# BimberLab/nimble

Measured on NVIDIA B200. Metric: reads/sec (device-timed, 1/2/4/8 B200) vs MHC-like lib; SW GCUPS; HBM GB/s, higher is better.
Workload: dtype u64 k-mers / s16x2 DPX / f64 thresholds

## Files before the change

### nimble_b200/csrc/kernels.cuh

```cuda
#pragma once
#include <cstddef>
#include <cstdint>
#include <cuda_runtime.h>

#include "../../include/nimble_b200.h"
#include "kmer_hash.hpp"

namespace nb200 {

constexpr int kBand = 8;
constexpr int kNB = 2 * kBand + 1;
constexpr int kVW = 64;
constexpr uint32_t kXP = 0xFF7FFF7Fu;
constexpr uint32_t kGP = 0xFF3FFF3Fu;
constexpr uint32_t kMatchDelta = 193;
constexpr uint32_t kInvalid = 0xFFFFFFFFu;
constexpr int kCap = 32;
constexpr int kScratchWords = 16 * kCap;
constexpr uint32_t kFull = 0xFFFFFFFFu;
constexpr int kProbeWarps = 2;

struct LibDev {
    const uint4 *table;
    uint32_t n_buckets;
// ... 479 lines not shown
};

__device__ __forceinline__ bool candidate_round(const LibDev &lib, const int o, const uint32_t cl, uint32_t cap, int lane, uint32_t *lw, uint32_t *lb,
                                                int &na, int &owner, bool &dead, OwnerB &B) {
    const bool hit = cl != kInvalid;
    uint4 c_b, c_w;
    ldg256_cached(lib.class_rec + 2 * (size_t)(hit ? cl : 0u), c_b, c_w);
    const bool inl = (int32_t)c_w.z >= 0;
    if (na < 0) {
        const uint32_t cn = inl ? (c_w.z & 0xFFu) : c_b.y;
        const uint32_t m = __reduce_min_sync(kFull, hit ? ((min(cn, 0x3FFFFFFu) << 5) | (uint32_t)lane) : kInvalid);
        const int src = (int)(m & 31);
        const uint32_t nn = m >> 5;
        if (nn > cap) return false;
        na = (int)nn;
        if (nn <= 4 && owner < 0) {
            owner = o;
            B.w01 = __shfl_sync(kFull, c_w.x, src); B.w23 = __shfl_sync(kFull, c_w.y, src);
            B.b0 = __shfl_sync(kFull, c_b.x, src); B.b1 = __shfl_sync(kFull, c_b.y, src);
            B.b2 = __shfl_sync(kFull, c_b.z, src); B.b3 = __shfl_sync(kFull, c_b.w, src);
        } else {
            anchor_to_list(lib, lw, lb, nn, c_b, c_w, src, lane);
        }
    }
    if (o == owner) {
        const bool same = !hit || (c_w.x == B.w01 && c_w.y == B.w23 && inl);
        if (__all_sync(kFull, same)) {
            if (hit) { B.a0 &= c_b.x; B.a1 &= c_b.y; B.a2 &= c_b.z; B.a3 &= c_b.w; }
        } else {
            if (hit && inl) {
                B.a0 &= rec_bits(lib, c_b, c_w, B.w01 & 0xFFFFu);
                B.a1 &= rec_bits(lib, c_b, c_w, B.w01 >> 16);
                B.a2 &= rec_bits(lib, c_b, c_w, B.w23 & 0xFFFFu);
                B.a3 &= rec_bits(lib, c_b, c_w, B.w23 >> 16);
            }
            bool ovf = hit && !inl;
            while (__any_sync(kFull, ovf)) {
                if (ovf) {
#pragma unroll 1
                    for (int j = 0; j < na; j++) {
                        const uint32_t word = j == 0 ? (B.w01 & 0xFFFFu) : (j == 1 ? (B.w01 >> 16) : (j == 2 ? (B.w23 & 0xFFFFu) : (B.w23 >> 16)));
                        const uint32_t v = rec_lookup_overflow(lib.ov_w, lib.ov_b, c_b.x, c_b.y, word);
                        if (j == 0) B.a0 &= v; else if (j == 1) B.a1 &= v; else if (j == 2) B.a2 &= v; else B.a3 &= v;
                    }
                }
                ovf = false;
            }
        }
    } else if (!intersect_generic(lib, lw, lb, na, hit, c_b, c_w, lane)) {
        dead = true;
    }
    return true;
}

template <bool kStats>
__device__ __forceinline__ bool probe_mate(const LibDev &lib, const ReadsDev &R, uint64_t read, int lane, uint32_t cap,
                                           List *lists , MateProbe &M, uint32_t &n_probe, uint32_t &slots_read) {
    const uint8_t *rec = R.packed + read * R.stride;
    const int W = (int)R.words;
    const int L = read_length(R, read);
    const int k = lib.k;
    const int P = L - k + 1;
    M.L = L; M.P = P;
    const uint32_t kmask_lo = (uint32_t)lib.kmask, kmask_hi = (uint32_t)(lib.kmask >> 32), kbits = (uint32_t)lib.kbits;
    const int rshift = 64 - 2 * k;
    const uint32_t nb = lib.n_buckets;
    uint32_t nh0 = 0, nh1 = 0;
    int seed_i0 = -1, seed_i1 = -1;
    int na0 = -1, na1 = -1, owner = -1;
    bool dead0 = false, dead1 = false;
    OwnerB B;
    B.w01 = B.w23 = 0xFFFFFFFFu; B.b0 = B.b1 = B.b2 = B.b3 = 0; B.a0 = B.a1 = B.a2 = B.a3 = kFull;
    uint32_t my_lo = 0, my_hi = 0, my_n = 0;
    if (lane < W && P > 0) {
        const uint2 v = *reinterpret_cast<const uint2 *>(rec + (size_t)lane * 8);
        my_lo = v.x; my_hi = v.y;
        my_n = *reinterpret_cast<const uint32_t *>(rec + (size_t)W * 8 + (size_t)lane * 4);
    }
    uint32_t w0 = __shfl_sync(kFull, my_lo, 0), w1 = __shfl_sync(kFull, my_hi, 0), n_lo = __shfl_sync(kFull, my_n, 0);
    const bool upper = lane >= 16;
    const int n_rounds = P > 0 ? (P + 31) >> 5 : 0;

#pragma unroll 1
    for (int r = 0; r < n_rounds; r++) {
        const int i = (r << 5) + lane;
        const uint32_t w2 = __shfl_sync(kFull, my_lo, r + 1), w3 = __shfl_sync(kFull, my_hi, r + 1), n_hi = __shfl_sync(kFull, my_n, r + 1);
        const uint32_t ea = upper ? w1 : w0, eb = upper ? w2 : w1, ec = upper ? w3 : w2;
        const uint32_t x_lo = __funnelshift_r(ea, eb, 2 * lane) & kmask_lo;
        const uint32_t x_hi = __funnelshift_r(eb, ec, 2 * lane) & kmask_hi;
        const bool valid = i < P && (__funnelshift_r(n_lo, n_hi, lane) & kbits) == 0;
        w0 = w2; w1 = w3; n_lo = n_hi;
        uint32_t p_lo = __brev(~x_hi), p_hi = __brev(~x_lo);
        p_lo = ((p_lo >> 1) & 0x55555555u) | ((p_lo << 1) & 0xAAAAAAAAu);
        p_hi = ((p_hi >> 1) & 0x55555555u) | ((p_hi << 1) & 0xAAAAAAAAu);
        const uint32_t y_lo = rshift >= 32 ? p_hi >> (rshift - 32) : __funnelshift_r(p_lo, p_hi, rshift);
        const uint32_t y_hi = rshift >= 32 ? 0u : p_hi >> rshift;
        const bool x_lt = x_hi < y_hi || (x_hi == y_hi && x_lo < y_lo), x_eq = x_hi == y_hi && x_lo == y_lo;
        const uint32_t c_lo = x_lt ? x_lo : y_lo, c_hi = x_lt ? x_hi : y_hi;
        const uint32_t mix = kmer_mix(c_lo, c_hi);
        const uint32_t b1 = valid ? kmer_bucket1(mix, nb) : 0u;
        uint4 e_lo, e_hi;
        ldg256(lib.table + 2 * (size_t)b1, e_lo, e_hi);
        bool m0 = e_lo.x == c_lo && e_lo.y == c_hi, m1 = e_hi.x == c_lo && e_hi.y == c_hi;
        const bool need2 = valid && !(m0 || m1) && (e_lo.z & kDevSpill);
        if (kStats) { n_probe += valid ? 1u : 0u; slots_read += (valid ? 1u : 0u) + (need2 ? 1u : 0u); }
        const bool xs = x_lt || x_eq, ys = !x_lt;
        uint32_t ecls = m0 ? e_lo.z : e_hi.z;
        bool found = valid && (m0 || m1);
        uint32_t cl0 = (found && xs != ((ecls & kDevRc) != 0)) ? (ecls & kDevIdMask) : kInvalid;
        uint32_t cl1 = (found && ys != ((ecls & kDevRc) != 0)) ? (ecls & kDevIdMask) : kInvalid;
        bool slow = need2 || (found && (ecls & kDevDual));
        while (__any_sync(kFull, slow)) {
            if (slow) {
                if (need2) {
                    ldg256(lib.table + 2 * (size_t)kmer_bucket2(mix, c_lo, b1, nb), e_lo, e_hi);
                    m0 = e_lo.x == c_lo && e_lo.y == c_hi; m1 = e_hi.x == c_lo && e_hi.y == c_hi;
                    found = m0 || m1;
                    ecls = m0 ? e_lo.z : e_hi.z;
                    cl0 = (found && xs != ((ecls & kDevRc) != 0)) ? (ecls & kDevIdMask) : kInvalid;
                    cl1 = (found && ys != ((ecls & kDevRc) != 0)) ? (ecls & kDevIdMask) : kInvalid;
                }
                if (found && (ecls & kDevDual)) {
                    const uint4 d = __ldg(lib.dual + (ecls & kDevIdMask));
                    cl0 = xs ? d.x : d.z;
                    cl1 = ys ? d.x : d.z;
                }
            }
            slow = false;
        }
        const unsigned hb0 = __ballot_sync(kFull, cl0 != kInvalid), hb1 = __ballot_sync(kFull, cl1 != kInvalid);
        if (hb0) {
            nh0 += __popc(hb0);
            if (seed_i0 < 0) seed_i0 = (r << 5) + __ffs(hb0) - 1;
            if (!dead0 && !candidate_round(lib, 0, cl0, cap, lane, lists[0].w, lists[0].b, na0, owner, dead0, B)) return false;
        }
        if (hb1) {
            nh1 += __popc(hb1);
            seed_i1 = P - 1 - ((r << 5) + 31 - __clz(hb1));
            if (!dead1 && !candidate_round(lib, 1, cl1, cap, lane, lists[1].w, lists[1].b, na1, owner, dead1, B)) return false;
        }
    }
    lists[0].n = na0 > 0 ? na0 : 0; lists[1].n = na1 > 0 ? na1 : 0;
    M.owner = owner;
    if (owner >= 0) {
        const int na = owner ? na1 : na0;
        M.reg.w01 = B.w01; M.reg.w23 = B.w23;
        M.reg.b0 = B.b0 & __reduce_and_sync(kFull, B.a0);
        M.reg.b1 = na > 1 ? B.b1 & __reduce_and_sync(kFull, B.a1) : 0u;
        M.reg.b2 = na > 2 ? B.b2 & __reduce_and_sync(kFull, B.a2) : 0u;
        M.reg.b3 = na > 3 ? B.b3 & __reduce_and_sync(kFull, B.a3) : 0u;
    }
    __syncwarp();
    M.nh[0] = nh0; M.nh[1] = nh1; M.seed_i[0] = seed_i0; M.seed_i[1] = seed_i1;
    return true;
}

__device__ __forceinline__ void owner_to_list(const MateProbe &M, List *lists, int lane) {
    if (M.owner < 0) return;
    List &Lo = lists[M.owner];
    if (lane < Lo.n) {
        Lo.w[lane] = lane == 0 ? (M.reg.w01 & 0xFFFFu) : (lane == 1 ? (M.reg.w01 >> 16) : (lane == 2 ? (M.reg.w23 & 0xFFFFu) : (M.reg.w23 >> 16)));
        Lo.b[lane] = lane == 0 ? M.reg.b0 : (lane == 1 ? M.reg.b1 : (lane == 2 ? M.reg.b2 : M.reg.b3));
    }
    __syncwarp();
}

__device__ __forceinline__ void emit_items(const LibDev &lib, const List &B, uint32_t seed_cls, uint32_t seed_off, int seed_i,
                                           uint32_t ro_idx, uint32_t len, uint32_t cnt, SwItem *items, uint32_t off, int lane) {
    const Rec seed = load_rec(lib, seed_cls);
    uint32_t run = 0;
    for (int base = 0; base < B.n; base += 32) {
        const int j = base + lane;
        const uint32_t bits = j < B.n ? B.b[j] : 0u, word = j < B.n ? B.w[j] : 0u;
        uint32_t tot;
        const uint32_t ex = warp_excl_scan(__popc(bits), lane, tot);
        const int nw = min(32, B.n - base);
        for (uint32_t c0 = 0; c0 < tot; c0 += 32) {
            const uint32_t c = c0 + lane;
            int owner = 0;
            for (int jj = 1; jj < nw; jj++) if (__shfl_sync(kFull, ex, jj) <= c) owner = jj;
            const uint32_t obits = __shfl_sync(kFull, bits, owner), oword = __shfl_sync(kFull, word, owner);
            const uint32_t oex = __shfl_sync(kFull, ex, owner);
            if (c < tot) {
                uint32_t rest = obits;
                for (uint32_t t = c - oex; t > 0; t--) rest &= rest - 1;
                const uint32_t r = oword * 32 + (uint32_t)(__ffs(rest) - 1);
                const uint32_t pos = __ldg(lib.positions + seed_off + rec_rank(lib, seed, r));
                SwItem it;
                it.ro = ro_idx | (len << kRoIdxBits); it.ref = r;
                it.gwin = __ldg(lib.ref_gstart + r) + pos - (uint32_t)seed_i - (uint32_t)kBand;
                it.v = 0;
                items[off + run + c] = it;
            }
        }
        run += tot;
    }
    if (lane == 0 && (cnt & 1)) {
        SwItem it; it.ro = ro_idx | (len << kRoIdxBits); it.ref = kInvalid; it.gwin = 0; it.v = 0;
        items[off + cnt] = it;
    }
}

__device__ __forceinline__ void carve_scratch(uint32_t *s, uint32_t cap, List *L4, List &T, List &Bst) {
#pragma unroll
    for (int q = 0; q < 4; q++) { L4[q].w = s + (size_t)q * 2 * cap; L4[q].b = L4[q].w + cap; L4[q].n = 0; }
    T.w = s + (size_t)8 * cap; T.b = T.w + 2 * (size_t)cap; T.n = 0;
    Bst.w = s + (size_t)12 * cap; Bst.b = Bst.w + 2 * (size_t)cap; Bst.n = 0;
}

template <int NM, bool kStats>
__device__ __forceinline__ void probe_read(const LibDev &lib, const ReadsDev &r1, const ReadsDev &r2, uint64_t read0, uint32_t gw,
                                           OriSum *__restrict__ sums, uint32_t *__restrict__ roB, uint32_t *__restrict__ wide_list,
                                           Counters *__restrict__ ctr, List *L4, int lane, uint32_t &n_probe, uint32_t &slots_read) {
    const uint64_t read = read0 + gw;
    constexpr int n_ro = NM * 2;
    bool wide = false;
#pragma unroll
    for (int m = 0; m < NM; m++) {
        if (wide) break;
        MateProbe M;
        if (!probe_mate<kStats>(lib, m ? r2 : r1, read, lane, lib.narrow_cap, &L4[m * 2], M, n_probe, slots_read)) { wide = true; break; }
#pragma unroll
        for (int o = 0; o < 2; o++) {
            const int q = m * 2 + o;
            const int na = L4[q].n;
            const bool in_mem = na > 4, reg = M.owner == o;
            const bool full = M.nh[o] && (int)M.nh[o] == M.P;
            uint32_t w01 = 0xFFFFFFFFu, w23 = 0xFFFFFFFFu, b0 = 0, b1 = 0, b2 = 0, b3 = 0;
            if (reg) { w01 = M.reg.w01; w23 = M.reg.w23; b0 = M.reg.b0; b1 = M.reg.b1; b2 = M.reg.b2; b3 = M.reg.b3; }
            else if (na > 0 && !in_mem) {
                const uint32_t *lw = L4[q].w, *lb = L4[q].b;
                const uint32_t x0 = lw[0], x1 = na > 1 ? lw[1] : 0xFFFFu, x2 = na > 2 ? lw[2] : 0xFFFFu, x3 = na > 3 ? lw[3] : 0xFFFFu;
                w01 = x0 | (x1 << 16); w23 = x2 | (x3 << 16);
                b0 = lb[0]; b1 = na > 1 ? lb[1] : 0u; b2 = na > 2 ? lb[2] : 0u; b3 = na > 3 ? lb[3] : 0u;
            } else if (in_mem) {
                uint32_t *dst = roB + ((size_t)gw * n_ro + q) * 2 * kCap;
                for (int j = lane; j < na; j += 32) { dst[j] = L4[q].w[j]; dst[kCap + j] = L4[q].b[j]; }
            }
            if (lane == 0) {
                uint4 *dst = reinterpret_cast<uint4 *>(sums + (size_t)gw * n_ro + q);
                const uint32_t flags = (full ? kSumFull : 0u) | (in_mem ? kSumInMem : 0u);
                dst[0] = make_uint4((M.nh[o] & 0xFFFFu) | ((uint32_t)(M.seed_i[o] & 0xFFFF) << 16),
                                    (uint32_t)na | (flags << 8) | ((uint32_t)M.L << 16), w01, w23);
                dst[1] = make_uint4(b0, b1, b2, b3);
            }
        }
    }
    if (wide && lane == 0) {
        wide_list[atomicAdd(&ctr->n_wide, 1ull)] = gw;
        reinterpret_cast<uint4 *>(sums + (size_t)gw * n_ro)[0] = make_uint4(0u, (uint32_t)kSumWide << 8, 0xFFFFFFFFu, 0xFFFFFFFFu);
    }
}

template <bool kStats>
__device__ __forceinline__ void add_probe_stats(Counters *ctr, int lane, uint32_t n_probe, uint32_t slots_read) {
    if (!kStats) return;
    n_probe = warp_sum(n_probe);
    slots_read = warp_sum(slots_read);
    if (lane == 0 && n_probe) {
        atomicAdd(&ctr->probes[blockIdx.x & (kCtrSpread - 1)], (unsigned long long)n_probe);
        atomicAdd(&ctr->probe_slots[blockIdx.x & (kCtrSpread - 1)], (unsigned long long)slots_read);
    }
}

__device__ __forceinline__ void carve_probe_lists(uint32_t *smem, int wib, List *L4) {
#pragma unroll
    for (int q = 0; q < 4; q++) { L4[q].w = smem + ((size_t)wib * 4 + q) * 2 * kCap; L4[q].b = L4[q].w + kCap; L4[q].n = 0; }
}

template <int NM, bool kStats>
__global__ void __launch_bounds__(kProbeWarps * 32, (NM == 2 ? 24 : 36) / kProbeWarps)
probe_kernel(LibDev lib, ReadsDev r1, ReadsDev r2, uint64_t read0, uint64_t n_reads, OriSum *__restrict__ sums,
             uint32_t *__restrict__ roB, uint32_t *__restrict__ wide_list, Counters *__restrict__ ctr) {
    __shared__ uint32_t smem[kProbeWarps * 4 * 2 * kCap];
    const int lane = threadIdx.x & 31, wib = threadIdx.x >> 5;
    const uint32_t gw = blockIdx.x * kProbeWarps + wib;
    if (gw >= n_reads) return;
    List L4[4];
    carve_probe_lists(smem, wib, L4);
    uint32_t n_probe = 0, slots_read = 0;
    probe_read<NM, kStats>(lib, r1, r2, read0, gw, sums, roB, wide_list, ctr, L4, lane, n_probe, slots_read);
    add_probe_stats<kStats>(ctr, lane, n_probe, slots_read);
}

constexpr int kProbeListBlocks = 24 / kProbeWarps;
template <bool kStats>
__global__ void __launch_bounds__(kProbeWarps * 32, kProbeListBlocks)
probe_list_kernel(LibDev lib, ReadsDev r1, uint64_t read0, const uint32_t *__restrict__ warp_list, OriSum *__restrict__ sums,
                  uint32_t *__restrict__ roB, uint32_t *__restrict__ wide_list, Counters *__restrict__ ctr) {
    __shared__ uint32_t smem[kProbeWarps * 4 * 2 * kCap];
    const int lane = threadIdx.x & 31, wib = threadIdx.x >> 5;
    const uint32_t n = (uint32_t)ctr->n_probe_warp;
    List L4[4];
    carve_probe_lists(smem, wib, L4);
    uint32_t n_probe = 0, slots_read = 0;
    for (uint32_t t = blockIdx.x * kProbeWarps + wib; t < n; t += gridDim.x * kProbeWarps) {
        __syncwarp();
        probe_read<1, kStats>(lib, r1, r1, read0, warp_list[t], sums, roB, wide_list, ctr, L4, lane, n_probe, slots_read);
    }
    add_probe_stats<kStats>(ctr, lane, n_probe, slots_read);
}

constexpr int kProbeThreads = 128;
constexpr int kProbeGroup = 1;
constexpr int kProbeThreadBlocks = 10;

struct ThreadB {
    uint32_t nh, prev;
    int seed;
};
enum { SB_NA = 0, SB_W01, SB_W23, SB_B0, SB_B1, SB_B2, SB_B3, SB_N };
#define NB200_SB(f) sb[(f) * kProbeThreads]

__device__ __forceinline__ bool thread_hit(const LibDev &lib, ThreadB &T, uint32_t *sb, uint32_t cl, int i, int o, uint32_t cap,
                                           const uint4 c_b, const uint4 c_w) {
    T.nh++;
    if (o == 0) T.seed = T.seed < 0 ? i : T.seed; else T.seed = i;
    if (cl == T.prev) return true;
    const bool inl = (int32_t)c_w.z >= 0;
    if (T.prev == kInvalid) {
        T.prev = cl;
        const uint32_t na = c_w.z & 0xFFu;
        NB200_SB(SB_NA) = na;
        if (!inl || na > cap) return false;
        NB200_SB(SB_W01) = c_w.x; NB200_SB(SB_W23) = c_w.y;
        NB200_SB(SB_B0) = c_b.x; NB200_SB(SB_B1) = c_b.y; NB200_SB(SB_B2) = c_b.z; NB200_SB(SB_B3) = c_b.w;
        return true;
    }
    T.prev = cl;
    const uint32_t w01 = NB200_SB(SB_W01), w23 = NB200_SB(SB_W23);
    uint4 m = c_b;
    if (!(inl && c_w.x == w01 && c_w.y == w23)) {
        m.x = rec_bits(lib, c_b, c_w, w01 & 0xFFFFu);
        m.y = rec_bits(lib, c_b, c_w, w01 >> 16);
        m.z = rec_bits(lib, c_b, c_w, w23 & 0xFFFFu);
        m.w = rec_bits(lib, c_b, c_w, w23 >> 16);
    }
    NB200_SB(SB_B0) &= m.x; NB200_SB(SB_B1) &= m.y; NB200_SB(SB_B2) &= m.z; NB200_SB(SB_B3) &= m.w;
    return true;
}

template <bool kStats>
__global__ void __launch_bounds__(kProbeThreads, kProbeThreadBlocks)
probe_thread_kernel(LibDev lib, ReadsDev R, uint64_t read0, uint64_t n_reads, OriSum *__restrict__ sums,
                    uint32_t *__restrict__ warp_list, Counters *__restrict__ ctr) {
    const uint32_t gr = blockIdx.x * kProbeThreads + threadIdx.x;
    const bool active = gr < n_reads;
    const uint64_t read = read0 + (active ? gr : 0u);
    const uint8_t *rec = R.packed + read * R.stride;
    const uint64_t *seq = reinterpret_cast<const uint64_t *>(rec);
    const int W = (int)R.words, k = lib.k;
    const int P = (active ? read_length(R, read) : 0) - k + 1;
    const uint64_t kmask = lib.kmask;
    const int top = 2 * k - 2;
    const uint32_t nb = lib.n_buckets, cap = min(4u, lib.narrow_cap);
    __shared__ uint32_t s_b[2 * SB_N * kProbeThreads];
    uint32_t *const sb0 = s_b + threadIdx.x, *const sb1 = sb0 + SB_N * kProbeThreads;
    ThreadB T[2];
#pragma unroll
    for (int o = 0; o < 2; o++) {
        uint32_t *sb = o ? sb1 : sb0;
        T[o].nh = 0; T[o].prev = kInvalid; T[o].seed = -1;
        NB200_SB(SB_NA) = 0; NB200_SB(SB_W01) = NB200_SB(SB_W23) = 0xFFFFFFFFu;
        NB200_SB(SB_B0) = NB200_SB(SB_B1) = NB200_SB(SB_B2) = NB200_SB(SB_B3) = 0;
    }
    uint32_t n_probe = 0, slots_read = 0;
    bool fallback = false;
    uint64_t cur = 0, x = 0, y = 0;
    uint32_t ncur = 0;
    int p = 0, last_n = -1;
    auto push_base = [&]() {
        if ((p & 31) == 0) {
            const int w = p >> 5;
            cur = w < W ? seq[w] : 0ull;
            ncur = w < W ? reinterpret_cast<const uint32_t *>(seq + W)[w] : 0u;
        }
        const uint32_t b = (uint32_t)cur & 3u;
        last_n = (ncur & 1u) ? p : last_n;
        cur >>= 2; ncur >>= 1;
        x = (x >> 2) | ((uint64_t)b << top);
        y = ((y << 2) | (b ^ 3u)) & kmask;
        p++;
    };
    if (P > 0)
        for (int t = 0; t < k - 1; t++) push_base();
#pragma unroll 1
    for (int i0 = 0; i0 < P; i0 += kProbeGroup) {
        uint32_t c_lo[kProbeGroup], c_hi[kProbeGroup];
        bool valid[kProbeGroup], xs[kProbeGroup], ys[kProbeGroup];
        uint4 e_lo[kProbeGroup], e_hi[kProbeGroup];
#pragma unroll
        for (int g = 0; g < kProbeGroup; g++) {
            push_base();
            const int i = i0 + g;
            valid[g] = i < P && last_n < i;
            const bool x_lt = x < y;
            xs[g] = x <= y; ys[g] = !x_lt;
            const uint64_t c = x_lt ? x : y;
            c_lo[g] = (uint32_t)c; c_hi[g] = (uint32_t)(c >> 32);
            e_lo[g] = make_uint4(kInvalid, kInvalid, 0u, 0u); e_hi[g] = e_lo[g];
            if (valid[g]) ldg256(lib.table + 2 * (size_t)kmer_bucket1(kmer_mix(c_lo[g], c_hi[g]), nb), e_lo[g], e_hi[g]);
        }
        uint32_t cl0[kProbeGroup], cl1[kProbeGroup];
#pragma unroll
        for (int g = 0; g < kProbeGroup; g++) {
            const uint32_t clo = c_lo[g], chi = c_hi[g];
            bool m0 = e_lo[g].x == clo && e_lo[g].y == chi, m1 = e_hi[g].x == clo && e_hi[g].y == chi;
            uint32_t ecls = m0 ? e_lo[g].z : e_hi[g].z;
            bool found = valid[g] && (m0 || m1);
            const bool need2 = valid[g] && !(m0 || m1) && (e_lo[g].z & kDevSpill);
            if (kStats) { n_probe += valid[g] ? 1u : 0u; slots_read += (valid[g] ? 1u : 0u) + (need2 ? 1u : 0u); }
            if (need2 || (found && (ecls & kDevDual))) {
                if (need2) {
                    const uint32_t mix = kmer_mix(clo, chi);
                    uint4 f_lo, f_hi;
                    ldg256(lib.table + 2 * (size_t)kmer_bucket2(mix, clo, kmer_bucket1(mix, nb), nb), f_lo, f_hi);
                    m0 = f_lo.x == clo && f_lo.y == chi; m1 = f_hi.x == clo && f_hi.y == chi;
                    found = m0 || m1;
                    ecls = m0 ? f_lo.z : f_hi.z;
                }
                cl0[g] = (found && xs[g] != ((ecls & kDevRc) != 0)) ? (ecls & kDevIdMask) : kInvalid;
                cl1[g] = (found && ys[g] != ((ecls & kDevRc) != 0)) ? (ecls & kDevIdMask) : kInvalid;
                if (found && (ecls & kDevDual)) {
                    const uint4 d = __ldg(lib.dual + (ecls & kDevIdMask));
                    cl0[g] = xs[g] ? d.x : d.z;
                    cl1[g] = ys[g] ? d.x : d.z;
                }
            } else {
                cl0[g] = (found && xs[g] != ((ecls & kDevRc) != 0)) ? (ecls & kDevIdMask) : kInvalid;
                cl1[g] = (found && ys[g] != ((ecls & kDevRc) != 0)) ? (ecls & kDevIdMask) : kInvalid;
            }
        }
        uint4 r_b[kProbeGroup], r_w[kProbeGroup];
        uint32_t r_cl[kProbeGroup];
        {
            uint32_t p0 = T[0].prev, p1 = T[1].prev;
#pragma unroll
            for (int g = 0; g < kProbeGroup; g++) {
                const bool n0 = cl0[g] != kInvalid && cl0[g] != p0, n1 = cl1[g] != kInvalid && cl1[g] != p1;
                r_cl[g] = n0 ? cl0[g] : (n1 ? cl1[g] : kInvalid);
                if (cl0[g] != kInvalid) p0 = cl0[g];
                if (cl1[g] != kInvalid) p1 = cl1[g];
                r_b[g] = make_uint4(0u, 0u, 0u, 0u); r_w[g] = r_b[g];
                if (r_cl[g] != kInvalid) ldg256_cached(lib.class_rec + 2 * (size_t)r_cl[g], r_b[g], r_w[g]);
            }
        }
#pragma unroll
        for (int g = 0; g < kProbeGroup; g++) {
            if (cl0[g] != kInvalid && !thread_hit(lib, T[0], sb0, cl0[g], i0 + g, 0, cap, r_b[g], r_w[g])) fallback = true;
            if (cl1[g] != kInvalid) {
                uint4 c_b = r_b[g], c_w = r_w[g];
                if (cl1[g] != T[1].prev && cl1[g] != r_cl[g]) ldg256_cached(lib.class_rec + 2 * (size_t)cl1[g], c_b, c_w);
                if (!thread_hit(lib, T[1], sb1, cl1[g], i0 + g, 1, cap, c_b, c_w)) fallback = true;
            }
        }
        if (fallback) break;
    }
    const unsigned fb = __ballot_sync(kFull, active && fallback);
    if (fb) {
        const int lane = threadIdx.x & 31, leader = __ffs(fb) - 1;
        uint32_t base = 0;
        if (lane == leader) base = (uint32_t)atomicAdd(&ctr->n_probe_warp, (unsigned long long)__popc(fb));
        base = __shfl_sync(kFull, base, leader);
        if (active && fallback) warp_list[base + __popc(fb & ((1u << lane) - 1))] = gr;
    }
    if (fallback) n_probe = slots_read = 0;
    add_probe_stats<kStats>(ctr, threadIdx.x & 31, n_probe, slots_read);
    if (!active || fallback) return;
    uint4 *dst = reinterpret_cast<uint4 *>(sums + (size_t)gr * 2);
#pragma unroll
    for (int o = 0; o < 2; o++) {
        const ThreadB &B = T[o];
        const uint32_t *sb = o ? sb1 : sb0;
        const uint32_t na = B.prev == kInvalid ? 0u : NB200_SB(SB_NA);
        const int seed = B.nh == 0 ? -1 : (o == 0 ? B.seed : P - 1 - B.seed);
        const uint32_t flags = (B.nh && (int)B.nh == P) ? kSumFull : 0u;
        dst[2 * o] = make_uint4((B.nh & 0xFFFFu) | ((uint32_t)(seed & 0xFFFF) << 16), na | (flags << 8) | ((uint32_t)(P + k - 1) << 16),
                                NB200_SB(SB_W01), NB200_SB(SB_W23));
        dst[2 * o + 1] = make_uint4(NB200_SB(SB_B0), na > 1 ? NB200_SB(SB_B1) : 0u, na > 2 ? NB200_SB(SB_B2) : 0u,
                                    na > 3 ? NB200_SB(SB_B3) : 0u);
    }
}
#undef NB200_SB

struct SmallList { uint32_t w[8], b[8]; int n; };

__device__ __forceinline__ void small_from_sum(const uint4 lo, const uint4 hi, SmallList &A) {
    A.n = (int)(lo.y & 0xFFu);
    A.w[0] = lo.z & 0xFFFFu; A.w[1] = lo.z >> 16; A.w[2] = lo.w & 0xFFFFu; A.w[3] = lo.w >> 16;
    A.b[0] = hi.x; A.b[1] = hi.y; A.b[2] = hi.z; A.b[3] = hi.w;
}
__device__ __forceinline__ uint32_t small_count(const SmallList &A) {
    uint32_t c = 0;
    for (int j = 0; j < A.n; j++) c += __popc(A.b[j]);
    return c;
}

template <int NM>
__device__ __forceinline__ int thread_call(const LibDev &lib, const CallParams &cp, const uint4 (&lo)[NM * 2], const uint4 (&hi)[NM * 2],
                                           const uint32_t (&nh)[4], const uint32_t (&nc)[4], const int (&len)[4], const int (&vbest)[4],
                                           uint32_t n_sw, int32_t *fout, uint32_t *rec) {
    constexpr int n_ro = NM * 2;
    constexpr bool paired = NM == 2;
    const int mh = cp.max_hits;
    int n_feat = 0;
    int st[4] = {ST_NONE, ST_NONE, ST_NONE, ST_NONE}, sc[4] = {0, 0, 0, 0}, ed[4] = {0, 0, 0, 0};
#pragma unroll
    for (int o = 0; o < n_ro; o++) {
        if (nh[o] == 0) { st[o] = ST_NO_MATCH; continue; }
        if (vbest[o] < 0) { st[o] = ST_EMPTY; continue; }
        sc[o] = (vbest[o] + kVW - 1) / kVW;
        ed[o] = sc[o] * kVW - vbest[o];
        if (sc[o] < cp.score_threshold) st[o] = ST_SCORE;
        else if (sc[o] < (int)cp.min_score[len[o]]) st[o] = ST_PERCENT;
        else if (cp.discard_multiple_matches && nc[o] > 1) st[o] = ST_MULTI;
        else st[o] = ST_PASS;
    }
    const bool any_pass = st[0] == ST_PASS || st[1] == ST_PASS || st[2] == ST_PASS || st[3] == ST_PASS;
    int chosen = -1, chosen_max = 0;
    int first_fail = (!any_pass && paired && cp.require_valid_pair) ? RS_NOT_VALID_PAIR : RS_NO_PASS;
    uint32_t chosen_score = 0;
    int reason, n_feat_local = 0;
    if constexpr (!paired) {
        const bool en0 = any_pass && cp.strand_filter != NB200_THREEPRIME, en1 = any_pass && cp.strand_filter != NB200_FIVEPRIME;
        if (en0 && st[0] == ST_PASS) { chosen = 0; chosen_score = (uint32_t)sc[0]; }
        if (en1 && st[1] == ST_PASS && (chosen < 0 || (uint32_t)sc[1] > chosen_score)) { chosen = 1; chosen_score = (uint32_t)sc[1]; }
        chosen_max = (int)chosen_score;
        reason = first_fail;
        if (chosen >= 0) {
            const uint4 l = chosen ? lo[1] : lo[0], h = chosen ? hi[1] : hi[0];
            const int n = (int)(l.y & 0xFFu);
            const uint32_t w0 = l.z & 0xFFFFu, w1 = l.z >> 16, w2 = l.w & 0xFFFFu, w3 = l.w >> 16;
            const uint32_t b0 = h.x, b1 = n > 1 ? h.y : 0u, b2 = n > 2 ? h.z : 0u, b3 = n > 3 ? h.w : 0u;
            if (chosen_max < cp.score_filter) reason = RS_SCORE_FILTER;
            else {
                const bool ident = lib.identity != 0;
                int nf = 0;
                uint32_t prev = kInvalid;
                auto count_word = [&](uint32_t w, uint32_t bits) {
                    if (ident) { nf += __popc(bits); return; }
                    while (bits) {
                        const int bpos = __ffs(bits) - 1; bits &= bits - 1;
                        const uint32_t f = __ldg(lib.ref_feature + w * 32 + bpos);
                        if (f != prev) { nf++; prev = f; }
                    }
                };
                count_word(w0, b0); count_word(w1, b1); count_word(w2, b2); count_word(w3, b3);
                if (cp.discard_multi_hits > 0 && nf > cp.discard_multi_hits) reason = RS_MULTI_HITS;
                else if (nf > mh) reason = RS_MAX_HITS;
                else {
                    reason = RS_CALLED; n_feat_local = nf;
                    int at = 0;
                    prev = kInvalid;
                    auto emit_word = [&](uint32_t w, uint32_t bits) {
                        while (bits) {
                            const int bpos = __ffs(bits) - 1; bits &= bits - 1;
                            const uint32_t r = w * 32 + bpos;
                            const uint32_t f = ident ? r : __ldg(lib.ref_feature + r);
                            if (f != prev) { fout[at++] = (int32_t)f; prev = f; }
                        }
                    };
                    emit_word(w0, b0); emit_word(w1, b1); emit_word(w2, b2); emit_word(w3, b3);
                }
            }
        }
    } else {
    int order[4], n_cfg = 0;
    switch (any_pass ? cp.strand_filter : -1) {
    case -1: break;
    case NB200_FIVEPRIME: order[n_cfg++] = 0; break;
    case NB200_THREEPRIME: order[n_cfg++] = 1; break;
    case NB200_STRAND_NONE: order[n_cfg++] = 0; order[n_cfg++] = 1; order[n_cfg++] = 2; order[n_cfg++] = 3; break;
    default: order[n_cfg++] = 0; order[n_cfg++] = 1; break;
    }
    SmallList best;
    best.n = 0;
    for (int ci = 0; ci < n_cfg; ci++) {
        const int c = order[ci];
        const int ia = (c == 0 || c == 2) ? 0 : 1;
        const int ib = (c == 0 || c == 3) ? 3 : 2;
        const int sa = sc[ia], sbv = sc[ib];
        const bool pa = st[ia] == ST_PASS, pb = st[ib] == ST_PASS;
        int fail = -1, maxmate = 0;
        uint32_t sum = 0;
        SmallList cur;
        cur.n = 0;
        if (cp.require_valid_pair && !(pa && pb)) fail = RS_NOT_VALID_PAIR;
        else if (!pa && !pb) fail = RS_NO_PASS;
        else if (pa && pb) {
            sum = (uint32_t)(sa + sbv); maxmate = max(sa, sbv);
            SmallList A, Bl;
            small_from_sum(lo[ia], hi[ia], A); small_from_sum(lo[ib], hi[ib], Bl);
            if (cp.intersect_level == 0) {
                int i = 0, j = 0, n = 0;
                while (i < A.n || j < Bl.n) {
                    if (j >= Bl.n || (i < A.n && A.w[i] < Bl.w[j])) { cur.w[n] = A.w[i]; cur.b[n] = A.b[i]; i++; }
                    else if (i >= A.n || Bl.w[j] < A.w[i]) { cur.w[n] = Bl.w[j]; cur.b[n] = Bl.b[j]; j++; }
                    else { cur.w[n] = A.w[i]; cur.b[n] = A.b[i] | Bl.b[j]; i++; j++; }
                    n++;
                }
                cur.n = n;
            } else {
                uint32_t any = 0;
                for (int i = 0; i < A.n; i++) {
                    uint32_t v = 0;
                    for (int j = 0; j < Bl.n; j++) if (Bl.w[j] == A.w[i]) v = Bl.b[j];
                    cur.w[i] = A.w[i]; cur.b[i] = A.b[i] & v;
                    any |= cur.b[i];
                }
                cur.n = A.n;
                if (!any) {
                    if (cp.intersect_level >= 2) fail = RS_FORCE_INTERSECT;
                    else if (sbv > sa) cur = Bl; else cur = A;
                }
            }
        } else {
            if (cp.intersect_level >= 2) fail = RS_FORCE_INTERSECT;
            else { sum = (uint32_t)(pa ? sa : sbv); maxmate = (int)sum; small_from_sum(pa ? lo[ia] : lo[ib], pa ? hi[ia] : hi[ib], cur); }
        }
        if (fail >= 0) { if (ci == 0) first_fail = fail; continue; }
        if (chosen < 0 || sum > chosen_score) { chosen = c; chosen_score = sum; chosen_max = maxmate; best = cur; }
    }
    reason = first_fail;
    if (chosen >= 0) {
        if (chosen_max < cp.score_filter) reason = RS_SCORE_FILTER;
        else if (lib.identity) {
            const int nf = (int)small_count(best);
            if (cp.discard_multi_hits > 0 && nf > cp.discard_multi_hits) reason = RS_MULTI_HITS;
            else if (nf > mh) reason = RS_MAX_HITS;
            else {
                reason = RS_CALLED; n_feat_local = nf;
                int at = 0;
                for (int j = 0; j < best.n; j++) {
                    uint32_t bits = best.b[j];
                    while (bits) { const int bpos = __ffs(bits) - 1; bits &= bits - 1; fout[at++] = (int32_t)(best.w[j] * 32 + bpos); }
                }
            }
        } else {
            int nf = 0;
            uint32_t prev = kInvalid;
            for (int j = 0; j < best.n; j++) {
                uint32_t bits = best.b[j];
                while (bits) {
                    const int bpos = __ffs(bits) - 1; bits &= bits - 1;
                    const uint32_t f = __ldg(lib.ref_feature + best.w[j] * 32 + bpos);
                    if (f != prev) { nf++; prev = f; }
                }
            }
            if (cp.discard_multi_hits > 0 && nf > cp.discard_multi_hits) reason = RS_MULTI_HITS;
            else if (nf > mh) reason = RS_MAX_HITS;
            else {
                reason = RS_CALLED; n_feat_local = nf;
                int at = 0;
                prev = kInvalid;
                for (int j = 0; j < best.n; j++) {
                    uint32_t bits = best.b[j];
                    while (bits) {
                        const int bpos = __ffs(bits) - 1; bits &= bits - 1;
                        const uint32_t f = __ldg(lib.ref_feature + best.w[j] * 32 + bpos);
                        if (f != prev) { fout[at++] = (int32_t)f; prev = f; }
                    }
                }
            }
        }
    }
    }
    n_feat = n_feat_local;
    for (int t = n_feat; t < mh; t++) fout[t] = -1;
    static_assert(sizeof(nb200_read_result) == 40 && offsetof(nb200_read_result, n_hits) == 8 && offsetof(nb200_read_result, n_cand) == 16 &&
                  offsetof(nb200_read_result, edits) == 24 && offsetof(nb200_read_result, status) == 28 &&
                  offsetof(nb200_read_result, reason) == 32 && offsetof(nb200_read_result, pair_score) == 36,
                  "the word-wise stores follow the layout of nb200_read_result");
    auto c16 = [](uint32_t v) { return v > 65535u ? 65535u : v; };
    rec[0] = (uint32_t)sc[0] | ((uint32_t)sc[1] << 16); rec[1] = (uint32_t)sc[2] | ((uint32_t)sc[3] << 16);
    rec[2] = nh[0] | (nh[1] << 16); rec[3] = nh[2] | (nh[3] << 16);
    rec[4] = c16(nc[0]) | (c16(nc[1]) << 16); rec[5] = c16(nc[2]) | (c16(nc[3]) << 16);
    rec[6] = (uint32_t)ed[0] | ((uint32_t)ed[1] << 8) | ((uint32_t)ed[2] << 16) | ((uint32_t)ed[3] << 24); rec[7] = (uint32_t)st[0] | ((uint32_t)st[1] << 8) | ((uint32_t)st[2] << 16) | ((uint32_t)st[3] << 24);
    rec[8] = (uint32_t)reason | ((uint32_t)(chosen < 0 ? 255 : chosen) << 8) | ((uint32_t)n_feat << 16) | (n_sw << 24);
    rec[9] = chosen < 0 ? 0u : chosen_score;
    return n_feat;
}

constexpr int kFastThreads = 256;
template <int NM>
__global__ void __launch_bounds__(kFastThreads)
call_fast_kernel(LibDev lib, CallParams cp, const OriSum *__restrict__ sums, uint32_t n_reads, uint32_t *__restrict__ slow_list,
                 uint32_t *__restrict__ setup_list, nb200_read_result *__restrict__ results, int32_t *__restrict__ feats,
                 uint16_t *__restrict__ row_nf, Counters *__restrict__ ctr) {
    constexpr int n_ro = NM * 2;
    constexpr bool paired = NM == 2;
    const uint32_t gw = blockIdx.x * blockDim.x + threadIdx.x;
    const int lane = threadIdx.x & 31;
    bool active = gw < n_reads, slow = false, inmem = false;
    uint4 lo[n_ro], hi[n_ro];
    if (active) {
        const uint4 *src = reinterpret_cast<const uint4 *>(sums + (size_t)gw * n_ro);
#pragma unroll
        for (int q = 0; q < n_ro; q++) { lo[q] = __ldg(src + 2 * q); hi[q] = __ldg(src + 2 * q + 1); }
        if ((lo[0].y >> 8) & kSumWide) active = false;
    }
    uint32_t nh[4] = {0, 0, 0, 0}, nc[4] = {0, 0, 0, 0};
    int len[4] = {0, 0, 0, 0};
    if (active) {
#pragma unroll
        for (int q = 0; q < n_ro; q++) {
            nh[q] = lo[q].x & 0xFFFFu; len[q] = (int)(lo[q].y >> 16);
            const uint32_t flags = (lo[q].y >> 8) & 0xFFu;
            const int na = (int)(lo[q].y & 0xFFu);
            if (flags & kSumInMem) { slow = true; inmem = true; continue; }
            uint32_t c = 0;
            if (na > 0) c = __popc(hi[q].x) + (na > 1 ? __popc(hi[q].y) : 0) + (na > 2 ? __popc(hi[q].z) : 0) + (na > 3 ? __popc(hi[q].w) : 0);
            nc[q] = c;
            if (nh[q] && c && !(flags & kSumFull)) slow = true;
        }
    }
    const bool setup = slow && !inmem;
    slow = slow && inmem;
    __shared__ uint32_t s_cnt[2][kFastThreads / 32];
    unsigned sb = 0, ub = 0;
    uint32_t my_base = 0;
    {
        sb = __ballot_sync(kFull, active && slow); ub = __ballot_sync(kFull, active && setup);
        if (lane == 0) { s_cnt[0][threadIdx.x >> 5] = __popc(sb); s_cnt[1][threadIdx.x >> 5] = __popc(ub); }
        __syncthreads();
        if (threadIdx.x < 2) {
            uint32_t tot = 0;
#pragma unroll
            for (int w = 0; w < kFastThreads / 32; w++) tot += s_cnt[threadIdx.x][w];
            my_base = tot ? (uint32_t)atomicAdd(threadIdx.x ? &ctr->n_setup : &ctr->n_slow, (unsigned long long)tot) : 0u;
        }
    }
    slow = slow || setup;
    extern __shared__ uint32_t stage[];
    const int mh = cp.max_hits;
    const int wib = threadIdx.x >> 5;
    uint32_t *s_res = stage + (size_t)wib * 32 * (10 + mh), *s_feat = s_res + 32 * 10;
    const bool mine = active && !slow;
    const unsigned okmask = __ballot_sync(kFull, mine);
    int n_feat = 0;
    if (mine) {
        int vbest[4];
#pragma unroll
        for (int o = 0; o < 4; o++) vbest[o] = nc[o] ? len[o] * kVW : -1;
        n_feat = thread_call<NM>(lib, cp, lo, hi, nh, nc, len, vbest, 0u, reinterpret_cast<int32_t *>(s_feat) + lane * mh, s_res + lane * 10);
        row_nf[gw] = (uint16_t)n_feat;
    }
    __syncwarp();
    const uint32_t gw0 = gw - (uint32_t)lane;
    if (okmask) {
        uint2 *dst = reinterpret_cast<uint2 *>(results + gw0);
        const uint2 *src = reinterpret_cast<const uint2 *>(s_res);
        for (int t = lane; t < 32 * 5; t += 32)
            if ((okmask >> (t / 5)) & 1u) dst[t] = src[t];
        int32_t *fd = feats + (size_t)gw0 * mh;
        for (int t = lane; t < 32 * mh; t += 32)
            if ((okmask >> (t / mh)) & 1u) fd[t] = (int32_t)s_feat[t];
    }
    {
        __shared__ uint32_t s_base[2];
        if (threadIdx.x < 2) s_base[threadIdx.x] = my_base;
// ... 724 lines not shown
```

Measured before the change: 586.7 million.

## Decouple class-record intersection via per-thread shared-memory queue in thread probe kernel

```diff
diff --git a/nimble_b200/csrc/kernels.cuh b/nimble_b200/csrc/kernels.cuh
--- a/nimble_b200/csrc/kernels.cuh
+++ b/nimble_b200/csrc/kernels.cuh
@@ -805,8 +805,11 @@
 }
 
 constexpr int kProbeThreads = 128;
-constexpr int kProbeGroup = 1;
+constexpr int kProbeGroup = 2;
+constexpr int kProbeQueue = 16;
+constexpr int kQueueSlots = kProbeQueue + 2 * kProbeGroup - 1;
 constexpr int kProbeThreadBlocks = 10;
+constexpr uint32_t kQueueOri = 1u << 30, kQueueAnchor = 1u << 31;
 
 struct ThreadB {
     uint32_t nh, prev;
@@ -815,14 +818,9 @@
 enum { SB_NA = 0, SB_W01, SB_W23, SB_B0, SB_B1, SB_B2, SB_B3, SB_N };
 #define NB200_SB(f) sb[(f) * kProbeThreads]
 
-__device__ __forceinline__ bool thread_hit(const LibDev &lib, ThreadB &T, uint32_t *sb, uint32_t cl, int i, int o, uint32_t cap,
-                                           const uint4 c_b, const uint4 c_w) {
-    T.nh++;
-    if (o == 0) T.seed = T.seed < 0 ? i : T.seed; else T.seed = i;
-    if (cl == T.prev) return true;
+__device__ __forceinline__ bool thread_and(const LibDev &lib, uint32_t *sb, uint32_t e, uint32_t cap, const uint4 c_b, const uint4 c_w) {
     const bool inl = (int32_t)c_w.z >= 0;
-    if (T.prev == kInvalid) {
-        T.prev = cl;
+    if (e & kQueueAnchor) {
         const uint32_t na = c_w.z & 0xFFu;
         NB200_SB(SB_NA) = na;
         if (!inl || na > cap) return false;
@@ -830,7 +828,6 @@
         NB200_SB(SB_B0) = c_b.x; NB200_SB(SB_B1) = c_b.y; NB200_SB(SB_B2) = c_b.z; NB200_SB(SB_B3) = c_b.w;
         return true;
     }
-    T.prev = cl;
     const uint32_t w01 = NB200_SB(SB_W01), w23 = NB200_SB(SB_W23);
     uint4 m = c_b;
     if (!(inl && c_w.x == w01 && c_w.y == w23)) {
@@ -841,6 +838,51 @@
     }
     NB200_SB(SB_B0) &= m.x; NB200_SB(SB_B1) &= m.y; NB200_SB(SB_B2) &= m.z; NB200_SB(SB_B3) &= m.w;
     return true;
+}
+
+__device__ __forceinline__ bool thread_drain(const LibDev &lib, const uint32_t *sq, int nq, uint32_t *sb0, uint32_t cap) {
+#pragma unroll 1
+    for (int j = 0; j < nq; j += 2) {
+        const bool two = j + 1 < nq;
+        const uint32_t e0 = sq[j * kProbeThreads], e1 = two ? sq[(j + 1) * kProbeThreads] : e0;
+        uint4 b0, w0, b1, w1;
+        ldg256_cached(lib.class_rec + 2 * (size_t)(e0 & kDevIdMask), b0, w0);
+        ldg256_cached(lib.class_rec + 2 * (size_t)(e1 & kDevIdMask), b1, w1);
+        if (!thread_and(lib, sb0 + ((e0 & kQueueOri) ? SB_N * kProbeThreads : 0), e0, cap, b0, w0)) return false;
+        if (two && !thread_and(lib, sb0 + ((e1 & kQueueOri) ? SB_N * kProbeThreads : 0), e1, cap, b1, w1)) return false;
+    }
+    return true;
+}
+
+template <bool kStats>
+__device__ __forceinline__ void bucket_classes(const LibDev &lib, bool valid, bool xs, bool ys, uint32_t clo, uint32_t chi,
+                                               const uint4 e_lo, const uint4 e_hi, uint32_t &cl0, uint32_t &cl1,
+                                               uint32_t &n_probe, uint32_t &slots_read) {
+    bool m0 = e_lo.x == clo && e_lo.y == chi, m1 = e_hi.x == clo && e_hi.y == chi;
+    uint32_t ecls = m0 ? e_lo.z : e_hi.z;
+    bool found = valid && (m0 || m1);
+    const bool need2 = valid && !(m0 || m1) && (e_lo.z & kDevSpill);
+    if (kStats) { n_probe += valid ? 1u : 0u; slots_read += (valid ? 1u : 0u) + (need2 ? 1u : 0u); }
+    if (need2 || (found && (ecls & kDevDual))) {
+        if (need2) {
+            const uint32_t mix = kmer_mix(clo, chi);
+            uint4 f_lo, f_hi;
+            ldg256(lib.table + 2 * (size_t)kmer_bucket2(mix, clo, kmer_bucket1(mix, lib.n_buckets), lib.n_buckets), f_lo, f_hi);
+            m0 = f_lo.x == clo && f_lo.y == chi; m1 = f_hi.x == clo && f_hi.y == chi;
+            found = m0 || m1;
+            ecls = m0 ? f_lo.z : f_hi.z;
+        }
+        cl0 = (found && xs != ((ecls & kDevRc) != 0)) ? (ecls & kDevIdMask) : kInvalid;
+        cl1 = (found && ys != ((ecls & kDevRc) != 0)) ? (ecls & kDevIdMask) : kInvalid;
+        if (found && (ecls & kDevDual)) {
+            const uint4 d = __ldg(lib.dual + (ecls & kDevIdMask));
+            cl0 = xs ? d.x : d.z;
+            cl1 = ys ? d.x : d.z;
+        }
+    } else {
+        cl0 = (found && xs != ((ecls & kDevRc) != 0)) ? (ecls & kDevIdMask) : kInvalid;
+        cl1 = (found && ys != ((ecls & kDevRc) != 0)) ? (ecls & kDevIdMask) : kInvalid;
+    }
 }
 
 template <bool kStats>
@@ -858,7 +900,9 @@
     const int top = 2 * k - 2;
     const uint32_t nb = lib.n_buckets, cap = min(4u, lib.narrow_cap);
     __shared__ uint32_t s_b[2 * SB_N * kProbeThreads];
-    uint32_t *const sb0 = s_b + threadIdx.x, *const sb1 = sb0 + SB_N * kProbeThreads;
+    __shared__ uint32_t s_q[kQueueSlots * kProbeThreads];
+    uint32_t *const sb0 = s_b + threadIdx.x, *const sb1 = sb0 + SB_N * kProbeThreads, *const sq = s_q + threadIdx.x;
+    int nq = 0;
     ThreadB T[2];
 #pragma unroll
     for (int o = 0; o < 2; o++) {
@@ -885,10 +929,29 @@
         y = ((y << 2) | (b ^ 3u)) & kmask;
         p++;
     };
-    if (P > 0)
+    const int Pw = __reduce_max_sync(kFull, P);
+    if (Pw > 0)
         for (int t = 0; t < k - 1; t++) push_base();
+    auto enqueue = [&](int i, uint32_t cl0, uint32_t cl1) {
+        if (cl0 != kInvalid) {
+            T[0].nh++;
+            T[0].seed = T[0].seed < 0 ? i : T[0].seed;
+            if (cl0 != T[0].prev) {
+                sq[nq++ * kProbeThreads] = cl0 | (T[0].prev == kInvalid ? kQueueAnchor : 0u);
+                T[0].prev = cl0;
+            }
+        }
+        if (cl1 != kInvalid) {
+            T[1].nh++;
+            T[1].seed = i;
+            if (cl1 != T[1].prev) {
+                sq[nq++ * kProbeThreads] = cl1 | kQueueOri | (T[1].prev == kInvalid ? kQueueAnchor : 0u);
+                T[1].prev = cl1;
+            }
+        }
+    };
 #pragma unroll 1
-    for (int i0 = 0; i0 < P; i0 += kProbeGroup) {
+    for (int i0 = 0; i0 < Pw; i0 += kProbeGroup) {
         uint32_t c_lo[kProbeGroup], c_hi[kProbeGroup];
         bool valid[kProbeGroup], xs[kProbeGroup], ys[kProbeGroup];
         uint4 e_lo[kProbeGroup], e_hi[kProbeGroup];
@@ -904,61 +967,18 @@
             e_lo[g] = make_uint4(kInvalid, kInvalid, 0u, 0u); e_hi[g] = e_lo[g];
             if (valid[g]) ldg256(lib.table + 2 * (size_t)kmer_bucket1(kmer_mix(c_lo[g], c_hi[g]), nb), e_lo[g], e_hi[g]);
         }
-        uint32_t cl0[kProbeGroup], cl1[kProbeGroup];
 #pragma unroll
         for (int g = 0; g < kProbeGroup; g++) {
-            const uint32_t clo = c_lo[g], chi = c_hi[g];
-            bool m0 = e_lo[g].x == clo && e_lo[g].y == chi, m1 = e_hi[g].x == clo && e_hi[g].y == chi;
-            uint32_t ecls = m0 ? e_lo[g].z : e_hi[g].z;
-            bool found = valid[g] && (m0 || m1);
-            const bool need2 = valid[g] && !(m0 || m1) && (e_lo[g].z & kDevSpill);
-            if (kStats) { n_probe += valid[g] ? 1u : 0u; slots_read += (valid[g] ? 1u : 0u) + (need2 ? 1u : 0u); }
-            if (need2 || (found && (ecls & kDevDual))) {
-                if (need2) {
-                    const uint32_t mix = kmer_mix(clo, chi);
-                    uint4 f_lo, f_hi;
-                    ldg256(lib.table + 2 * (size_t)kmer_bucket2(mix, clo, kmer_bucket1(mix, nb), nb), f_lo, f_hi);
-                    m0 = f_lo.x == clo && f_lo.y == chi; m1 = f_hi.x == clo && f_hi.y == chi;
-                    found = m0 || m1;
-                    ecls = m0 ? f_lo.z : f_hi.z;
-                }
-                cl0[g] = (found && xs[g] != ((ecls & kDevRc) != 0)) ? (ecls & kDevIdMask) : kInvalid;
-                cl1[g] = (found && ys[g] != ((ecls & kDevRc) != 0)) ? (ecls & kDevIdMask) : kInvalid;
-                if (found && (ecls & kDevDual)) {
-                    const uint4 d = __ldg(lib.dual + (ecls & kDevIdMask));
-                    cl0[g] = xs[g] ? d.x : d.z;
-                    cl1[g] = ys[g] ? d.x : d.z;
-                }
-            } else {
-                cl0[g] = (found && xs[g] != ((ecls & kDevRc) != 0)) ? (ecls & kDevIdMask) : kInvalid;
-                cl1[g] = (found && ys[g] != ((ecls & kDevRc) != 0)) ? (ecls & kDevIdMask) : kInvalid;
-            }
-        }
-        uint4 r_b[kProbeGroup], r_w[kProbeGroup];
-        uint32_t r_cl[kProbeGroup];
-        {
-            uint32_t p0 = T[0].prev, p1 = T[1].prev;
-#pragma unroll
-            for (int g = 0; g < kProbeGroup; g++) {
-                const bool n0 = cl0[g] != kInvalid && cl0[g] != p0, n1 = cl1[g] != kInvalid && cl1[g] != p1;
-                r_cl[g] = n0 ? cl0[g] : (n1 ? cl1[g] : kInvalid);
-                if (cl0[g] != kInvalid) p0 = cl0[g];
-                if (cl1[g] != kInvalid) p1 = cl1[g];
-                r_b[g] = make_uint4(0u, 0u, 0u, 0u); r_w[g] = r_b[g];
-                if (r_cl[g] != kInvalid) ldg256_cached(lib.class_rec + 2 * (size_t)r_cl[g], r_b[g], r_w[g]);
-            }
-        }
-#pragma unroll
-        for (int g = 0; g < kProbeGroup; g++) {
-            if (cl0[g] != kInvalid && !thread_hit(lib, T[0], sb0, cl0[g], i0 + g, 0, cap, r_b[g], r_w[g])) fallback = true;
-            if (cl1[g] != kInvalid) {
-                uint4 c_b = r_b[g], c_w = r_w[g];
-                if (cl1[g] != T[1].prev && cl1[g] != r_cl[g]) ldg256_cached(lib.class_rec + 2 * (size_t)cl1[g], c_b, c_w);
-                if (!thread_hit(lib, T[1], sb1, cl1[g], i0 + g, 1, cap, c_b, c_w)) fallback = true;
-            }
-        }
-        if (fallback) break;
-    }
+            uint32_t cl0, cl1;
+            bucket_classes<kStats>(lib, valid[g], xs[g], ys[g], c_lo[g], c_hi[g], e_lo[g], e_hi[g], cl0, cl1, n_probe, slots_read);
+            enqueue(i0 + g, cl0, cl1);
+        }
+        if (__any_sync(kFull, nq >= kProbeQueue)) {
+            if (!fallback && nq && !thread_drain(lib, sq, nq, sb0, cap)) fallback = true;
+            nq = 0;
+        }
+    }
+    if (!fallback && nq && !thread_drain(lib, sq, nq, sb0, cap)) fallback = true;
     const unsigned fb = __ballot_sync(kFull, active && fallback);
     if (fb) {
         const int lane = threadIdx.x & 31, leader = __ffs(fb) - 1;
```

Measured after the change: 614.7 million (median of 6 runs). +4.8%, better.
